# wadx2019/rpo

Measured on AMD Instinct MI355X. Metric: env-steps/sec (whole node), SafeCartpole-v0 (CartSafe-v0) RPODDPG, rollout + one batch-256 constrained policy update per vector step, higher is better.
Workload: dtype f32; 1 GPU; CartSafe-v0 RPODDPG, 4096 vectorised envs per MI355X, scripts/cart_exp.py hyper-parameters, update batch 256 every vector step (reference cadence), replay capacity 20000 per env; envs_per_gpu=4096, global_envs=4096, update_batch=256, hip_graph=True, training_batch_projection=row-wise, rccl_ranks=0, collectives_in_graph=False, graphs_replayed_on_all_ranks=True, graph_capture_fell_back_to_eager=False

## Files before the change

### include/rpo_hip.h

```cpp
#ifndef RPO_HIP_H
#define RPO_HIP_H

#ifdef __cplusplus
extern "C" {
#endif

#define RPO_ABI_VERSION 6

#define RPO_ERR_ARG (-1)
#define RPO_ERR_NULL (-2)

#define RPO_CART_STATE_DIM 6
#define RPO_CART_ACTION_DIM 2
#define RPO_CART_INEQ 6
#define RPO_CART_ROW 24
#define RPO_CART_RING 32
#define RPO_CART_CONSTS_LEN 35

#define RPO_PEND_INTERNAL_DIM 4
#define RPO_PEND_OBS_DIM 5
#define RPO_PEND_ACTION_DIM 2
#define RPO_PEND_ROW 16
#define RPO_PEND_RING 16

// ... 64 lines not shown
#define RPO_EVAL_LEN_SHIFT 2
#define RPO_EVAL_LANE_STEPS 4194304
#define RPO_EVOPF_EVAL_LANE_STEPS 12288

#define RPO_TRACE_ALIGN 4
#define RPO_TRACE_TAIL 4
#define RPO_TRACE_REWARD 0
#define RPO_TRACE_DONE 1
#define RPO_TRACE_INEQ 2
#define RPO_TRACE_EQ 3
#define RPO_TRACE_MAX_BYTES 1073741824

#define RPO_CON_ALIGN 4

#define RPO_CURVE_LEN 16
#define RPO_CURVE_STEP 0
#define RPO_CURVE_EPISODES 1
#define RPO_CURVE_STATS 2
#define RPO_CURVE_LENGTH 12
#define RPO_CURVE_VIOL_STEPS 13
#define RPO_CURVE_NONFINITE 14
#define RPO_CURVE_WS 4096
#define RPO_CURVE_MAX_EPISODES 1048576

#define RPO_NOISE_NONE 0
#define RPO_NOISE_EXPLICIT 1
#define RPO_NOISE_PHILOX 2
#define RPO_NOISE_UNIFORM 3
#define RPO_NOISE_CLIP_ONLY 4

#define RPO_STREAM_RESET 1
#define RPO_STREAM_ACT 2
#define RPO_STREAM_SAMPLE 3
#define RPO_STREAM_POLICY 4
#define RPO_STREAM_EVOPF_DEMAND 5
#define RPO_STREAM_EVOPF_PRICE 6
#define RPO_STREAM_EVAL_OBS 7
#define RPO_STREAM_EVOPF_DAY 8

int rpo_abi_version(void);

#define RPO_TUNE_FWD_STREAM 0
#define RPO_TUNE_FWD_STREAM_WAVES 1
#define RPO_TUNE_BWD_ONEPASS 2
#define RPO_TUNE_GEMM_KSPLIT 3
#define RPO_TUNE_MLP_GEMM 4
#define RPO_TUNE_ROLLOUT_WIDE 5
#define RPO_ROLLOUT_STREAM_FROM 65536
#define RPO_TUNE_BWD_STREAM 6
#define RPO_TUNE_L1_MFMA 7
#define RPO_TUNE_EVOPF_PLACE 8
#define RPO_TUNE_FWD_BF16X3 9
#define RPO_TUNE_COUNT 10
int rpo_tuning(int key, int value);

int rpo_philox_fill(int n, unsigned* out, unsigned long long seed, unsigned id_base, unsigned index,
                    unsigned stream_tag, void* stream);

int rpo_philox_normal(int n, float* out, unsigned long long seed, unsigned id_base, unsigned salt,
                      unsigned stream_tag, const long long* ctrl, void* stream);


int rpo_cartsafe_reset(int n_envs, float* state, int* ep_len, float* ep_ret, const unsigned* ep_count,
                       unsigned long long seed, unsigned env_id_base, void* stream);

int rpo_cartsafe_step(int n_envs, float* state, const float* action, int* ep_len, float* ep_ret, unsigned* ep_count,
                      float* rows, long long cap_steps, float* stats, int stats_cap, long long* ctrl,
                      const float* consts_host, int partial, int max_episode_steps, int auto_reset,
                      float viol_thresh, unsigned long long seed, unsigned env_id_base, void* stream);

int rpo_cartsafe_act_project(int n, const float* ap_raw, const float* noise, float* action, int* iters,
                             int noise_mode, float eps_start, float eps_end, float eps_decay, float box_lo,
                             float box_hi, int max_steps, float corr_lr, float corr_eps, float corr_momentum,
                             const float* consts_host, int partial, unsigned long long seed, unsigned env_id_base,
                             const long long* ctrl, float* stats, int stats_cap, void* stream);

int rpo_cartsafe_complete_bwd(int n, const float* grad_action, float* grad_ap, const float* consts_host,
                              int partial, void* stream);

int rpo_cartsafe_resid(int n, const float* action, float* eq_resid, float* ineq_resid, const float* consts_host,
                       int partial, void* stream);

int rpo_cartsafe_ineq_partial_grad(int n, const float* action, float* step, const float* consts_host, int partial,
                                   void* stream);

int rpo_cartsafe_lagrangian(int n, const float* action, const float* nu, float scale, float* loss_out,
                            float* grad_action, float* grad_nu, const float* consts_host, int partial, void* stream);

int rpo_pendulum_reset(int n_envs, float* internal, float* obs, int* ep_len, float* ep_ret, const unsigned* ep_count,
                       unsigned long long seed, unsigned env_id_base, void* stream);

int rpo_pendulum_step(int n_envs, float* internal, float* obs, const float* action, int* ep_len, float* ep_ret,
                      unsigned* ep_count, float* rows, long long cap_steps, float* stats, int stats_cap,
                      long long* ctrl, int max_episode_steps, int auto_reset, float viol_thresh,
                      unsigned long long seed, unsigned env_id_base, void* stream);

int rpo_pendulum_act_project(int n, const float* obs, int obs_stride, const float* ap_raw, const float* noise,
                             float* action, int* iters, int noise_mode, float eps_start, float eps_end,
                             float eps_decay, float box_lo, float box_hi, int max_steps, float corr_lr,
                             float corr_eps, float corr_momentum, unsigned long long seed, unsigned env_id_base,
                             const long long* ctrl, float* stats, int stats_cap, void* stream);

#define RPO_PROJ_WS_WORDS 5408
#define RPO_PROJ_WS_GAVE_UP 529
int rpo_pendulum_project_batchref(int n, const float* obs, int obs_stride, const float* ap, float* action,
                                  int* iters_out, int max_steps, float corr_lr, float corr_eps, float corr_momentum,
// ... 524 lines not shown
```

### rpo_amd/csrc/common.h

```cpp
#pragma once
#include <hip/hip_runtime.h>
#include <stdint.h>

#include "../../include/rpo_hip.h"

#define RPO_BLOCK 256
#define RPO_WAVE 64
#define RPO_MAX_GRID 2048

#define RPO_LAUNCH_CHECK()                        \
    do {                                          \
        hipError_t e__ = hipGetLastError();       \
        if (e__ != hipSuccess) return (int)e__;   \
    } while (0)

extern int g_rpo_tune[RPO_TUNE_COUNT];
static inline int rpo_tune(int key) { return g_rpo_tune[key]; }

__device__ __forceinline__ float rpo_relu_bits(float x) {
    const int b = __float_as_int(x);
    return __int_as_float(b > 0 ? b : 0);
}

__device__ __forceinline__ float rpo_relu(float x) { return __builtin_elementwise_maximum(x, 0.0f); }

static inline int rpo_cu_count() {
    static int cached[64] = {0};
    int dev = 0;
    if (hipGetDevice(&dev) != hipSuccess || dev < 0 || dev >= 64) return 256;
    if (cached[dev] == 0) {
        int v = 0;
        cached[dev] = (hipDeviceGetAttribute(&v, hipDeviceAttributeMultiprocessorCount, dev) == hipSuccess && v > 0) ? v : 256;
    }
    return cached[dev];
}

static inline int rpo_grid_for(long long n, int per_block = RPO_BLOCK) {
    long long g = (n + per_block - 1) / per_block;
    if (g < 1) g = 1;
    if (g > RPO_MAX_GRID) g = RPO_MAX_GRID;
    return (int)g;
}

struct rpo_u4 {
    uint32_t x, y, z, w;
};

__host__ __device__ __forceinline__ rpo_u4 rpo_philox(uint64_t seed, uint32_t id, uint32_t index, uint32_t stream,
                                                       uint32_t sub = 0u) {
    uint32_t c0 = id, c1 = index, c2 = stream, c3 = sub;
    uint32_t k0 = (uint32_t)seed, k1 = (uint32_t)(seed >> 32);
#pragma unroll
    for (int r = 0; r < 10; ++r) {
        const uint64_t p0 = (uint64_t)0xD2511F53u * c0;
        const uint64_t p1 = (uint64_t)0xCD9E8D57u * c2;
        const uint32_t n0 = (uint32_t)(p1 >> 32) ^ c1 ^ k0;
        const uint32_t n1 = (uint32_t)p1;
        const uint32_t n2 = (uint32_t)(p0 >> 32) ^ c3 ^ k1;
        const uint32_t n3 = (uint32_t)p0;
        c0 = n0; c1 = n1; c2 = n2; c3 = n3;
        k0 += 0x9E3779B9u;
        k1 += 0xBB67AE85u;
    }
    return rpo_u4{c0, c1, c2, c3};
}

__host__ __device__ __forceinline__ float rpo_u01(uint32_t x) { return (float)(x >> 8) * 5.9604644775390625e-08f; }

__device__ __forceinline__ float rpo_normal(uint32_t a, uint32_t b) {
// ... 196 lines not shown
```

### rpo_amd/csrc/nsplit.hip

```cpp
#include <stdlib.h>

#include "cartsafe_dev.h"
#include "heads_dev.h"
#include "host_glue.h"
#include "mlp_bwd.h"
#include "nsplit_dev.h"
#include "pendulum_dev.h"
#include "rollout_args.h"
#include "rollout_env.h"

namespace {

using namespace rpo_mlp_dev;
using namespace rpo_host;

bool split_ok(const Mlp& m) {
    return m.E == 128 && m.H == 256 && !m.cat && m.hd <= 1 && m.S <= 6 && m.A <= 4 && m.n_out >= 1 && m.n_out <= 2 && m.Ws && m.W0 &&
           m.W1 && (m.A == 0 || m.Wa) && (m.n_out == 1 || m.W1b);
}

struct NsBlock { int tile, g; };
__device__ __forceinline__ NsBlock ns_block() {
    const int lin = (int)blockIdx.x + (int)gridDim.x * (int)blockIdx.y, T = (int)gridDim.y;
    return NsBlock{lin % T, lin / T};
// ... 669 lines not shown
        for (int c0 = b_lo; !two && c0 < b_hi; c0 += 64) {
            float hv[64], d0[64];
#pragma unroll
            for (int u = 0; u < 64; ++u) {
                const int bb = c0 + u < b_hi ? c0 + u : b_hi - 1;
                hv[u] = h1[(size_t)bb * H + j];
                d0[u] = dglob[(size_t)bb * dstride];
            }
#pragma unroll
            for (int u = 0; u < 64; ++u) {
                const bool ok = c0 + u < b_hi;
                const float h = ok ? hv[u] : 0.0f, a0 = ok ? d0[u] : 0.0f;
                gb0 += ns_dh(h, a0, 0.0f, w1a, w1b);
                const float hr = fmaxf(h, 0.0f);
                gw1a = fmaf(a0, hr, gw1a);
                gw1b = fmaf(0.0f, hr, gw1b);
            }
        }
        for (int c0 = b_lo; two && c0 < b_hi; c0 += 32) {
            float hv[32], d0[32], d1[32];
#pragma unroll
            for (int u = 0; u < 32; ++u) {
                const int bb = c0 + u < b_hi ? c0 + u : b_hi - 1;
                hv[u] = h1[(size_t)bb * H + j];
                d0[u] = dglob[(size_t)bb * dstride];
                d1[u] = two ? dglob[(size_t)bb * dstride + 1] : 0.0f;
            }
#pragma unroll
            for (int u = 0; u < 32; ++u) {
                const bool ok = c0 + u < b_hi;
                const float h = ok ? hv[u] : 0.0f, a0 = ok ? d0[u] : 0.0f, a1 = ok ? d1[u] : 0.0f;
                gb0 += ns_dh(h, a0, a1, w1a, w1b);
                const float hr = fmaxf(h, 0.0f);
                gw1a = fmaf(a0, hr, gw1a);
                gw1b = fmaf(a1, hr, gw1b);
            }
        }
        partial[part][0][o] = gb0; partial[part][1][o] = gw1a; partial[part][2][o] = gw1b;
    }
    __syncthreads();
    if (tid < 16) {
        const int o = tid, j = rb * 16 + o;
        const float nb0 = cur_b0 + (((partial[0][0][o] + partial[1][0][o]) + partial[2][0][o]) + partial[3][0][o]);
        const float nw1 = cur_w1 + (((partial[0][1][o] + partial[1][1][o]) + partial[2][1][o]) + partial[3][1][o]);
        gr.b0[j] = nb0;
        gr.W1[j] = nw1;
        gmax = fmaxf(fabsf(nb0), fabsf(nw1));
        if (two) {
            const float nw1b = cur_w1b + (((partial[0][2][o] + partial[1][2][o]) + partial[2][2][o]) + partial[3][2][o]);
            gr.W1b[j] = nw1b;
            gmax = fmaxf(gmax, fabsf(nw1b));
        }
    }
    if (rb == 0) {
        __syncthreads();
        float s0 = 0.0f, s1 = 0.0f;
        for (int b2 = tid; b2 < B; b2 += kThreads) {
            s0 += dglob[(size_t)b2 * dstride];
            if (two) s1 += dglob[(size_t)b2 * dstride + 1];
        }
        { float ss[2] = {s0, s1}; rpo_wave_reduce_many(ss, 0u); s0 = ss[0]; s1 = ss[1]; }
        float* red = smem + 256;
        if ((tid & 63) == 0) { red[(tid >> 6) * 2] = s0; red[(tid >> 6) * 2 + 1] = s1; }
        __syncthreads();
        if (tid == 0) {
            const float nb1 = cur_b1 + (((red[0] + red[2]) + red[4]) + red[6]);
            gr.b1[0] = nb1;
            gmax = fmaxf(gmax, fabsf(nb1));
            if (two) {
                const float nb1b = cur_b1b + (((red[1] + red[3]) + red[5]) + red[7]);
                gr.b1b[0] = nb1b;
                gmax = fmaxf(gmax, fabsf(nb1b));
            }
        }
    }
    return gmax;
}

__device__ __forceinline__ float ns_weight_role(const Mlp& net, const MlpGrad& gr, const float* h1, const float* x0,
                                                const float* dglob, int dstride, bool two, int B, int w, float* smem) {
    if (w < kW0Tiles) return ns_dw0_tile(net, gr.W0, h1, x0, dglob, dstride, two, B, w, smem);
    return ns_hv_block(net, gr, h1, dglob, dstride, two, B, w - kW0Tiles, smem);
}

constexpr int kBwdASmem = kRows * (256 + 4) + 16 + 4 * 16 * 16;

template <class L>
__device__ __forceinline__ void bwd_a_role(const SplitArgs& p, float* smem, int b, unsigned fused_consumers = 0u,
                                           unsigned fused_need = 0u, unsigned fused_need_critics = 0u) {
    constexpr int EIN = 128, H = 256, LDH = H + 4;
    const int T = (p.B + kRows - 1) / kRows, B = p.B;
    const int tid = threadIdx.x, lane = tid & 63, wave = tid >> 6, li = lane & 15, lg = lane >> 4;
    {
        const int k = b / (T * kNsGroups), rem = b - k * T * kNsGroups, g = rem / T, tile = rem - g * T;
        const int row0 = tile * kRows;
        const Mlp& net = p.critic[k];
        float* dh_s = smem;
        float* dq_s = smem + kRows * LDH;
        float* wpart = dq_s + 16;
        const int jw = wave * (H / 4), e = g * 16 + li;
        float wv[H / 16], hv[kRows];
#pragma unroll
        for (int ks = 0; ks < H / 16; ++ks) wv[ks] = net.W0[(size_t)(jw + ks * 4 + lg) * EIN + e];
        const float w1a = net.W1[tid];
        if (fused_consumers && fused_need_critics)
            ns_tile_wait(p.tile_sync + (T + tile) * kNsSyncStride, fused_need_critics, p.tile_sync + 3 * T * kNsSyncStride, 16);
#pragma unroll
        for (int r = 0; r < kRows; ++r) hv[r] = row0 + r < B ? p.h1[k][(size_t)(row0 + r) * H + tid] : 0.0f;
        const size_t xo = (size_t)(row0 + (tid >> 4)) * EIN + g * 16 + (tid & 15);
        const float x0v = row0 + (tid >> 4) < B ? p.x0[k][xo] : 0.0f;
        if (fused_consumers) {
            ns_tile_wait(p.tile_sync + (T + tile) * kNsSyncStride, fused_need, p.tile_sync + 3 * T * kNsSyncStride);
            ns_tile_passed(p.tile_sync, T, tile, fused_consumers);
        }
        if (tid < 64) {
            float dq = 0.0f, hub = 0.0f;
            if (tid < kRows && row0 + tid < B) {
                dq = ns_td_row<L>(p, k, row0 + tid, &hub);
                if (g == 0) p.dq[k][row0 + tid] = dq;
            }
            if (tid < kRows) dq_s[tid] = dq;
            const float sum = rpo_row16_sum_desc_lane0(hub);
            if (tid == 0 && g == 0) p.loss_partial[k * T + tile] = sum;
        }
        __syncthreads();
#pragma unroll
        for (int r = 0; r < kRows; ++r) dh_s[r * LDH + tid] = (hv[r] > 0.0f) ? dq_s[r] * w1a : 0.0f;
        __syncthreads();
        f32x4 acc = f32x4{0.0f, 0.0f, 0.0f, 0.0f};
#pragma unroll
        for (int ks = 0; ks < H / 16; ++ks) acc = mfma4(dh_s[li * LDH + jw + ks * 4 + lg], wv[ks], acc);
#pragma unroll
        for (int i = 0; i < 4; ++i) wpart[(wave * 16 + lg * 4 + i) * 16 + li] = acc[i];
        __syncthreads();
        {
            const int r = tid >> 4, ee = tid & 15;
            float v = wpart[(0 * 16 + r) * 16 + ee];
            v = wpart[(1 * 16 + r) * 16 + ee] + v;
            v = wpart[(2 * 16 + r) * 16 + ee] + v;
            v = wpart[(3 * 16 + r) * 16 + ee] + v;
            if (row0 + r < B) p.dx0[k][xo] = x0v > 0.0f ? v : 0.0f;
        }
    }
}

template <class L>
__global__ __launch_bounds__(kThreads) void split_critic_bwd_a_kernel(SplitArgs p) {
    __shared__ __attribute__((aligned(16))) float smem[kBwdASmem];
    bwd_a_role<L>(p, smem, blockIdx.x);
}

__device__ __forceinline__ void adam_prepare(int* step_dev, float beta1, float beta2) {
    const int s = step_dev[0] + 1;
    double* cache = reinterpret_cast<double*>(step_dev + 4);
    cache[0] = 1.0 - pow((double)beta1, (double)s);
    cache[1] = sqrt(1.0 - pow((double)beta2, (double)s));
    step_dev[1] = s;
    step_dev[0] = s;
}

__device__ __forceinline__ void bwd_b_bookkeeping(const SplitArgs& p) {
    if (threadIdx.x != 0) return;
    if (p.prep_step) adam_prepare(p.prep_step, p.prep_beta1, p.prep_beta2);
    if (p.clock_out) p.clock_out[0] += 1;
    if (p.updates_out) p.updates_out[RPO_CTRL_UPDATES] += 1;
}

template <class L>
__device__ __forceinline__ void bwd_b_role(const SplitArgs& p, float* smem, int bx, int k, int own_blocks) {
    if ((p.prep_step || p.clock_out || p.updates_out) && bx == own_blocks - 1) {
        if (k == 0) bwd_b_bookkeeping(p);
        return;
    }
    if (bx < kWeightBlocks) {
        gradmax_flush(p.gradmax, ns_weight_role(p.critic[k], p.critic_grad[k], p.h1[k], p.x0[k], p.dq[k], 1, false, p.B, bx, smem));
        return;
    }
    BwdArgs a{};
    a.net = p.critic[k];
    a.g = p.critic_grad[k];
    a.n = p.B;
    a.s = p.batch_out; a.s_stride = L::ROW;
    a.a = p.batch_out + L::A_OFF; a.a_stride = L::ROW;
    a.dx0 = p.dx0[k];
    a.param_grads = 1;
    a.first_layer_state_only = 0;
    gradmax_flush(p.gradmax, mlp_bwd_first_layer<128>(a, bx - kWeightBlocks));
}

template <class L>
__global__ __launch_bounds__(kThreads) void split_critic_bwd_b_kernel(SplitArgs p) {
    __shared__ __attribute__((aligned(16))) float smem[4 * 16 * 16];
    bwd_b_role<L>(p, smem, blockIdx.x, blockIdx.y, gridDim.x);
}

template <class L>
__global__ __launch_bounds__(kThreads) void split_critic_bwd_b_ride_kernel(SplitArgs p, CartConsts c, RideArgs<typename L::Env> r,
                                                                           int own_blocks) {
    __shared__ __attribute__((aligned(16))) float smem[4 * 16 * 16];
    if ((int)blockIdx.x < own_blocks) bwd_b_role<L>(p, smem, blockIdx.x, blockIdx.y, own_blocks);
    else if (blockIdx.y == 0) ride_tail<typename L::Env>(r, c, smem, blockIdx.x - own_blocks, gridDim.x - own_blocks);
}

}

extern "C" {

int rpo_mlp_split_supported(const rpo_mlp* net) { return net && split_ok(to_dev(net)) ? 1 : 0; }

int rpo_mlp_forward_split(int k, const rpo_mlp* const* nets, int n, const float* const* s, const int* s_stride,
                          const float* const* a, const int* a_stride, float* const* part, float* const* x0_save,
                          float* const* h1_save, void* stream) {
    if (k < 1 || k > 4 || n <= 0 || !nets || !s || !part) return RPO_ERR_ARG;
    SplitFwdArgs4 all{};
    for (int i = 0; i < k; ++i) {
        if (!nets[i] || !s[i] || !part[i]) return RPO_ERR_NULL;
        const Mlp m = to_dev(nets[i]);
        if (!split_ok(m) || (m.A > 0 && (!a || !a[i]))) return RPO_ERR_ARG;
        all.net[i] = SplitFwdArgs{m, n, s[i], s_stride[i], m.A > 0 ? a[i] : nullptr, m.A > 0 ? a_stride[i] : 0, part[i],
                                  x0_save ? x0_save[i] : nullptr, h1_save ? h1_save[i] : nullptr};
    }
    hipLaunchKernelGGL(mlp_forward_split_kernel, dim3(kNsGroups, (n + kRows - 1) / kRows, k), dim3(kNsThreads), 0,
                       (hipStream_t)stream, all);
    RPO_LAUNCH_CHECK();
    return 0;
}

int rpo_mlp_split_head(const rpo_mlp* net, int n, const float* part, float* out, int out_mode, float scale, float base,
                       void* stream) {
    if (!net || !part || !out || n <= 0) return RPO_ERR_NULL;
    const Mlp m = to_dev(net);
    if (!split_ok(m)) return RPO_ERR_ARG;
    hipLaunchKernelGGL(mlp_split_head_kernel, dim3((n * m.n_out + RPO_BLOCK - 1) / RPO_BLOCK), dim3(RPO_BLOCK), 0,
                       (hipStream_t)stream, m, n, part, out, out_mode, scale, base);
    RPO_LAUNCH_CHECK();
    return 0;
}

}

namespace {

struct CartPol {
    typedef CartRow L;
    static constexpr int NI = 6;
    __device__ static __forceinline__ float2 complete(const CartConsts& c, const float* obs, int i, float ap, long long t) {
        rpo_cart_dev::ActArgs a{};
        a.noise_mode = RPO_NOISE_NONE; a.max_steps = 0;
        int k;
        return rpo_cart_dev::cart_explore_project(a, c, i, ap, 0.0f, t, k);
    }
    __device__ static __forceinline__ float lagr(const CartConsts& c, float a0, float a1, const float* nu_p, float scale,
                                                 float (&dist)[6], float2& g) {
// ... 575 lines not shown
            v = wpart[(3 * 16 + r) * 16 + ee] + v;
            if (xlive) {
                v = x0v > 0.0f ? v : 0.0f;
                if (p.shared_embedding) v += cdx;
                p.dx0_a[xo] = v;
            }
        }
    }
}

constexpr int kPolDSmem = kRows * (256 + 4) + 32 + 4 * 16 * 16;

template <class ENV>
__global__ __launch_bounds__(kThreads) void split_policy_d_kernel(SplitArgs p, CartConsts c) {
    __shared__ __attribute__((aligned(16))) float smem[kPolDSmem];
    pol_d_role<ENV>(p, c, smem, blockIdx.x);
}

constexpr int kPolFrontSmem = kPolDSmem > kFrontSmem ? kPolDSmem : kFrontSmem;

template <class ENV>
__global__ __launch_bounds__(kThreads) void split_policy_front_kernel(SplitArgs p, CartConsts c, int with_a) {
    typedef typename ENV::L L;
    __shared__ __attribute__((aligned(16))) float smem[kPolFrontSmem];
    const int K = p.twin ? 2 : 1, T = (int)gridDim.y, z = (int)blockIdx.z;
    const int lin = (int)blockIdx.x + (int)gridDim.x * (int)blockIdx.y;
    const unsigned consumers = (unsigned)(kNsGroups * (K * (1 + with_a) + 1));
    if (z == with_a + 2 * K) {
        pol_d_role<ENV>(p, c, smem, lin, consumers, with_a ? (unsigned)kNsGroups : 0u, (unsigned)(kNsGroups * K));
        return;
    }
    if (z >= with_a + K) {
        pol_c_role(p, smem, (z - with_a - K) * T * kNsGroups + lin, consumers, (unsigned)(kNsGroups * K));
        ns_tile_arrive(p.tile_sync + (lin % T) * kNsSyncStride, 1u << 16);
        return;
    }
    if (threadIdx.x >= kNsThreads) return;
    NsLds<128>& lds = *reinterpret_cast<NsLds<128>*>(smem);
    float4* tile = reinterpret_cast<float4*>(reinterpret_cast<char*>(smem) + sizeof(NsLds<128>));
    const NsBlock nb = ns_block();
    unsigned* sync = p.tile_sync;
    if (z < with_a) {
        pol_a_role<L>(p, lds, tile, nb.tile * kRows, nb.g);
        ns_tile_arrive(sync + nb.tile * kNsSyncStride);
    } else {
        pol_b_role<ENV>(p, c, lds, tile, nb.tile, nb.g, z - with_a, with_a ? sync + nb.tile * kNsSyncStride : nullptr,
                        (unsigned)kNsGroups);
        ns_tile_arrive(sync + (T + nb.tile) * kNsSyncStride);
        if (with_a) ns_tile_passed(sync, T, nb.tile, consumers);
    }
}

template <class ENV>
__global__ __launch_bounds__(kThreads) void split_policy_e_kernel(SplitArgs p, int fl_blocks) {
    typedef typename ENV::L L;
    __shared__ __attribute__((aligned(16))) float smem[4 * 16 * 16];
    if (blockIdx.x < kWeightBlocks) {
        gradmax_flush(p.gradmax, ns_weight_role(p.actor, p.actor_grad, p.h1_a, p.x0_a, p.dout, 2, p.actor.n_out > 1, p.B,
                                                blockIdx.x, smem));
        return;
    }
    const int fb = blockIdx.x - kWeightBlocks;
    if (fb == fl_blocks) {
        const int tid = threadIdx.x, T = (p.B + kRows - 1) / kRows;
        if (tid < 8) {
            float sacc = 0.0f;
            for (int g = 0; g < T; ++g) sacc += p.lag_partial[g * 8 + tid];
            const float inv_b = 1.0f / (float)p.B;
            if (tid == 0) p.lag_out[0] = inv_b * sacc;
            else if (tid == 7) { if (!p.twin) p.lag_out[1] = inv_b * sacc; }
            else if (tid - 1 < ENV::NI) p.nu_grad[tid - 1] += inv_b * sacc;
        }
        if (tid >= 64 && tid < 67 && p.prep2_step[tid - 64]) adam_prepare(p.prep2_step[tid - 64], p.prep2_beta1[tid - 64], p.prep2_beta2[tid - 64]);
        if (tid == 128 && p.clock_out) p.clock_out[0] += 1;
        if (tid == 192 && p.updates_out) p.updates_out[RPO_CTRL_UPDATES] += 1;
        return;
    }
    BwdArgs a{};
    a.net = p.actor;
    a.g = p.actor_grad;
    a.n = p.B;
    a.s = p.batch_out; a.s_stride = L::ROW;
    a.dx0 = p.dx0_a;
    a.param_grads = 1;
    gradmax_flush(p.gradmax, mlp_bwd_first_layer<128>(a, fb));
}

}

namespace {

enum : unsigned {
    kNeedPolicy = 1u,
    kNeedCritics = 2u, kNeedTargets = 4u, kNeedCriticGrads = 8u, kNeedActorGrad = 16u,
    kNeedActor = 32u,
};

int to_args(const rpo_split_update* u, unsigned need, SplitArgs& a, CartConsts& c) {
    if (!u) return RPO_ERR_NULL;
    if (u->batch <= 0 || u->batch > kBwdMaxB || (u->env != 0 && u->env != 1)) return RPO_ERR_ARG;
    const int S = u->env == 0 ? 6 : 5, K = u->twin ? 2 : 1;
    a = SplitArgs{};
    a.twin = u->twin ? 1 : 0; a.B = u->batch;
    auto ok_actor = [&](const rpo_mlp* h, Mlp& m) {
        if (!h) return (int)RPO_ERR_NULL;
        m = to_dev(h);
        return (split_ok(m) && m.S == S && m.A == 0 && m.n_out == (u->twin ? 2 : 1)) ? 0 : (int)RPO_ERR_ARG;
    };
    auto ok_critic = [&](const rpo_mlp* h, Mlp& m) {
        if (!h) return (int)RPO_ERR_NULL;
        m = to_dev(h);
        return (split_ok(m) && m.S == S && m.A == 2 && m.n_out == 1) ? 0 : (int)RPO_ERR_ARG;
    };
    if (need & kNeedPolicy) {
        if (int e = u->twin ? ok_actor(u->actor, a.actor) : ok_actor(u->actor_target, a.actor_target)) return e;
    }
    if (need & kNeedActor) {
        if (int e = ok_actor(u->actor, a.actor)) return e;
    }
    if (need & kNeedCritics) {
        if (int e = ok_critic(u->critic1, a.critic[0])) return e;
        if (K == 2) if (int e = ok_critic(u->critic2, a.critic[1])) return e;
    }
    if (need & kNeedTargets) {
        if (int e = ok_critic(u->critic_target1, a.critic_target[0])) return e;
        if (K == 2) if (int e = ok_critic(u->critic_target2, a.critic_target[1])) return e;
    }
    if (need & kNeedCriticGrads) {
        if (!u->critic1_grad || (K == 2 && !u->critic2_grad)) return RPO_ERR_NULL;
        a.critic_grad[0] = grad_dev(u->critic1_grad);
// ... 174 lines not shown
int fused_args(const rpo_split_update* u, const rpo_rollout_rider* r, Variant v, int env, unsigned need, SplitArgs& a, CartConsts& c) {
    if (int e = ride_checks(u, r, v, true)) return e;
    if (!u) return RPO_ERR_NULL;
    if (u->env != env) return RPO_ERR_ARG;
    return to_args(u, need | actor_need(v), a, c);
}

dim3 fused_grid(const SplitArgs& a, const rpo_rollout_rider* r, Variant v, int planes) {
    return slab_grid(a, planes + (v == kRide ? ride_planes(r, tiles(a.B), 2) : (int)(v == kPol)));
}

int front(const rpo_split_update* u, const rpo_rollout_rider* r, Variant v, void* stream) {
    SplitArgs a; CartConsts c;
    if (int e = fused_args(u, r, v, 0, kNeedPolicy | kNeedCritics | kNeedTargets, a, c)) return e;
    if (!a.batch_out || !a.ctrl || !a.part_pi || !a.tile_sync) return RPO_ERR_NULL;
    if (int e = sample_check(a, RPO_ERR_NULL)) return e;
    if ((a.twin && !a.logp) || a.max_steps < 0 || !a.loss_partial || !critic_bufs(a, kBufAll)) return RPO_ERR_NULL;
    if (int e = pol_check(u, a, v)) return e;
    const dim3 grid = fused_grid(a, r, v, 1 + 3 * critics(a));
    if (v == kRide) return launch(kFrontRide, grid, kThreads, 0, stream, a, c, Ride{a, r});
    return launch(kFront, grid, kThreads, 0, stream, a, c, (int)(v == kPol));
}

int mid(const rpo_split_update* u, const rpo_rollout_rider* r, Variant v, void* stream) {
    SplitArgs a; CartConsts c;
    if (int e = fused_args(u, r, v, 1, kNeedCritics | kNeedTargets, a, c)) return e;
    if (!a.batch_out || !a.ctrl || !a.next_actions || !a.tile_sync || !a.loss_partial || (a.twin && !a.logp) || !critic_bufs(a, kBufAll))
        return RPO_ERR_NULL;
    if (int e = pol_check(u, a, v)) return e;
    const dim3 grid = fused_grid(a, r, v, 2 * critics(a));
    if (v == kRide) return launch(kMidRide, grid, kThreads, 0, stream, a, c, Ride{a, r});
    return launch(kMid, grid, kThreads, 0, stream, a, c, (int)(v == kPol));
}

int pfront(const rpo_split_update* u, const rpo_rollout_rider* r, Variant v, void* stream) {
    SplitArgs a; CartConsts c;
    if (int e = fused_args(u, r, v, 1, kNeedPolicy | kNeedCritics | kNeedTargets, a, c)) return e;
    if (!a.batch_out || !a.ctrl || !a.part_pi || !a.next_actions || !a.tile_sync || !a.loss_partial || !u->proj_ws || (a.twin && !a.logp))
        return RPO_ERR_NULL;
    if (int e = sample_check(a, RPO_ERR_ARG)) return e;
    if (a.max_steps < 0 || !proj_multi_fits(a.B, a.max_steps) || !proj_ws_ok(u->proj_ws, u->proj_store_mode)) return RPO_ERR_ARG;
    if (!critic_bufs(a, kBufAll)) return RPO_ERR_NULL;
    if (int e = pol_check(u, a, v)) return e;
    const dim3 grid = fused_grid(a, r, v, 2 + 3 * critics(a));
    if (v == kRide) return launch(kPfrontRide, grid, kThreads, 0, stream, a, c, Ride{a, r}, u->proj_ws, u->proj_store_mode);
    return launch(kPfront, grid, kThreads, 0, stream, a, c, (int)(v == kPol), u->proj_ws, u->proj_store_mode);
}

int bwd_b(const rpo_split_update* u, const rpo_rollout_rider* r, Variant v, void* stream) {
    SplitArgs a; CartConsts c;
    if (int e = ride_checks(u, r, v, false)) return e;
    if (int e = to_args(u, kNeedCritics | kNeedCriticGrads | actor_need(v), a, c)) return e;
    if (!a.batch_out || !critic_bufs(a, kBufBwd)) return RPO_ERR_NULL;
    const int own = bwd_b_blocks(a);
    if (v == kRide)
        return launch_env(kBwdBRide, u->env, dim3(own + (r->n_envs + kThreads - 1) / kThreads, critics(a)), kThreads, stream, a, c,
                          Ride{a, r}, own);
    return launch_env(kBwdB, u->env, dim3(own, critics(a)), kThreads, stream, a);
}

int policy_b(const rpo_split_update* u, int fused, int with_a, void* stream) {
    SplitArgs a; CartConsts c;
    if (int e = to_args(u, kNeedActor | kNeedCritics, a, c)) return e;
    if (!a.batch_out || !a.ctrl || (!a.part_pi && !a.part_pol) || !a.nu || !a.noise_out || !a.actions || !a.g_act || !a.lag_partial ||
        (a.twin ? (!a.raw || !a.logp) : !a.ap_det) || !critic_bufs(a, kBufFwd))
        return RPO_ERR_NULL;
    if (!fused) return launch_env(kPolicyB, u->env, slab_grid(a, critics(a)), kNsThreads, stream, a, c);
    if (!a.tile_sync || !a.da_part || !critic_bufs(a, kBufDx0) || !a.dx0_a || !a.dout || !a.x0_a || !a.h1_a) return RPO_ERR_NULL;
    return launch_env(kPolicyFront, u->env, slab_grid(a, with_a + 2 * critics(a) + 1), kThreads, stream, a, c, with_a);
}

}

extern "C" {

int rpo_split_critic_fwd_a(const rpo_split_update* u, void* stream) { return fwd_a(u, nullptr, kPlain, stream); }
int rpo_split_critic_fwd_a_ride(const rpo_split_update* u, const rpo_rollout_rider* r, void* stream) { return fwd_a(u, r, kRide, stream); }

int rpo_split_critic_fwd_b(const rpo_split_update* u, void* stream) { return fwd_b(u, nullptr, kPlain, stream); }
int rpo_split_critic_fwd_b_pol(const rpo_split_update* u, void* stream) { return fwd_b(u, nullptr, kPol, stream); }
int rpo_split_critic_fwd_b_ride(const rpo_split_update* u, const rpo_rollout_rider* r, void* stream) { return fwd_b(u, r, kRide, stream); }

int rpo_split_critic_front(const rpo_split_update* u, void* stream) { return front(u, nullptr, kPlain, stream); }
int rpo_split_critic_front_pol(const rpo_split_update* u, void* stream) { return front(u, nullptr, kPol, stream); }
int rpo_split_critic_front_ride(const rpo_split_update* u, const rpo_rollout_rider* r, void* stream) { return front(u, r, kRide, stream); }

int rpo_split_critic_mid(const rpo_split_update* u, void* stream) { return mid(u, nullptr, kPlain, stream); }
int rpo_split_critic_mid_pol(const rpo_split_update* u, void* stream) { return mid(u, nullptr, kPol, stream); }
int rpo_split_critic_mid_ride(const rpo_split_update* u, const rpo_rollout_rider* r, void* stream) { return mid(u, r, kRide, stream); }

int rpo_split_critic_pfront(const rpo_split_update* u, void* stream) { return pfront(u, nullptr, kPlain, stream); }
int rpo_split_critic_pfront_pol(const rpo_split_update* u, void* stream) { return pfront(u, nullptr, kPol, stream); }
int rpo_split_critic_pfront_ride(const rpo_split_update* u, const rpo_rollout_rider* r, void* stream) { return pfront(u, r, kRide, stream); }

int rpo_split_critic_bwd_b(const rpo_split_update* u, void* stream) { return bwd_b(u, nullptr, kPlain, stream); }
int rpo_split_critic_bwd_b_ride(const rpo_split_update* u, const rpo_rollout_rider* r, void* stream) { return bwd_b(u, r, kRide, stream); }

int rpo_split_policy_b(const rpo_split_update* u, void* stream) { return policy_b(u, 0, 0, stream); }
int rpo_split_policy_front(const rpo_split_update* u, void* stream) { return policy_b(u, 1, 1, stream); }
int rpo_split_policy_front_bc(const rpo_split_update* u, void* stream) { return policy_b(u, 1, 0, stream); }

int rpo_split_critic_bwd_a(const rpo_split_update* u, void* stream) {
    SplitArgs a; CartConsts c;
    if (int e = to_args(u, kNeedCritics | kNeedTargets, a, c)) return e;
    if (!a.batch_out || !a.loss_partial || (a.twin && !a.logp) || !critic_bufs(a, kBufAll)) return RPO_ERR_NULL;
    return launch_env(kBwdA, u->env, dim3(critics(a) * tiles(a.B) * kNsGroups), kThreads, stream, a);
}

int rpo_split_pend_head_project(const rpo_split_update* u, void* stream) {
    SplitArgs a; CartConsts c;
    if (int e = to_args(u, kNeedPolicy, a, c)) return e;
    if (u->env != 1 || a.max_steps < 0) return RPO_ERR_ARG;
    if (!a.batch_out || !a.ctrl || !a.part_pi || !a.next_actions || (a.twin && !a.logp)) return RPO_ERR_NULL;
    static_assert(kPmWords == RPO_PROJ_WS_WORDS && kPmGaveUp == RPO_PROJ_WS_GAVE_UP, "workspace layout");
    if (u->proj_ws && proj_multi_fits(a.B, a.max_steps))
        return project_multi(a, u->proj_ws, u->proj_store_mode, nullptr, nullptr, 0, stream);
    if (a.B <= 256) return launch(split_pend_head_project_wide_kernel, dim3(1), 1024, 0, stream, a);
    return launch(kProjectTall, dim3(1), (a.B + RPO_WAVE - 1) / RPO_WAVE * RPO_WAVE, ((size_t)a.B + 4) * sizeof(float), stream, a);
}

int rpo_pendulum_project_batchref_ws(int n, const float* obs, int obs_stride, const float* ap, float* action, int* iters_out,
                                     int max_steps, float corr_lr, float corr_eps, float corr_momentum,
                                     unsigned long long* ws, int store_mode, void* stream) {
    if (n <= 0 || max_steps < 0 || !proj_multi_fits(n, max_steps) || obs_stride < RPO_PEND_OBS_DIM) return RPO_ERR_ARG;
    if (!obs || !ap || !action || !ws) return RPO_ERR_NULL;
    SplitArgs a{};
    a.B = n; a.next_actions = action; a.proj_iters = iters_out; a.max_steps = max_steps; a.corr_lr = corr_lr;
    a.corr_eps = corr_eps; a.corr_momentum = corr_momentum;
    return project_multi(a, ws, store_mode, ap, obs, obs_stride, stream);
}

int rpo_split_policy_a(const rpo_split_update* u, void* stream) {
    SplitArgs a; CartConsts c;
    if (int e = to_args(u, kNeedActor, a, c)) return e;
    if (!a.batch_out || (!a.part_pi && !a.part_pol) || !a.x0_a || !a.h1_a) return RPO_ERR_NULL;
    return launch_env(kPolicyA, u->env, dim3(kNsGroups, tiles(a.B)), kNsThreads, stream, a);
}

int rpo_split_policy_c(const rpo_split_update* u, void* stream) {
    SplitArgs a; CartConsts c;
    if (int e = to_args(u, kNeedCritics, a, c)) return e;
    if (!a.da_part || !a.lag_partial || (a.twin && !a.logp) || !critic_bufs(a, kBufFwd | kBufDx0)) return RPO_ERR_NULL;
    return launch(split_policy_c_kernel, dim3(critics(a) * tiles(a.B) * kNsGroups), kThreads, 0, stream, a);
}

int rpo_split_policy_d(const rpo_split_update* u, void* stream) {
    SplitArgs a; CartConsts c;
    if (int e = to_args(u, kNeedActor | kNeedActorGrad, a, c)) return e;
    if (!a.batch_out || !a.ctrl || !a.da_part || !a.g_act || !a.noise_out || !a.x0_a || !a.h1_a || !a.dx0_a || !a.dout ||
        (a.twin ? !a.raw : !a.ap_det) || (a.shared_embedding && !critic_bufs(a, kBufDx0)))
        return RPO_ERR_NULL;
    return launch_env(kPolicyD, u->env, dim3(tiles(a.B) * kNsGroups), kThreads, stream, a, c);
}

int rpo_split_policy_e(const rpo_split_update* u, void* stream) {
    SplitArgs a; CartConsts c;
    if (int e = to_args(u, kNeedActor | kNeedActorGrad, a, c)) return e;
    if (!a.batch_out || !a.dx0_a || !a.lag_partial || !a.lag_out || !a.nu_grad || !a.dout || !a.x0_a || !a.h1_a) return RPO_ERR_NULL;
    const int fl_blocks = mlp_fl_blocks(a.actor.E * (a.actor.S + 1));
    return launch_env(kPolicyE, u->env, dim3(kWeightBlocks + fl_blocks + 1), kThreads, stream, a, fl_blocks);
}

int rpo_xcc_probe(int gx, int gy, int gz, int threads, int* out, void* stream) {
    if (gx <= 0 || gy <= 0 || gz <= 0 || threads <= 0 || threads > 1024) return RPO_ERR_ARG;
    if (!out) return RPO_ERR_NULL;
    return launch(xcc_probe_kernel, dim3(gx, gy, gz), threads, 0, stream, out);
}

int rpo_hw_probe(int gx, int gy, int gz, int threads, int lds_bytes, int spin, int* out, void* stream) {
    if (gx <= 0 || gy <= 0 || gz <= 0 || threads <= 0 || threads > 1024 || lds_bytes < 4 || lds_bytes > 65536 || spin < 0) return RPO_ERR_ARG;
    if (!out) return RPO_ERR_NULL;
    return launch(hw_probe_kernel, dim3(gx, gy, gz), threads, lds_bytes, stream, out, spin);
}

}
```

### rpo_amd/csrc/train_ops.hip

```cpp
#include <stdlib.h>
#include "common.h"
#include "heads_dev.h"

namespace {

__global__ __launch_bounds__(RPO_BLOCK) void td_huber_kernel(
    int n, const float* __restrict__ q1, const float* __restrict__ q2, const float* __restrict__ qn1,
    const float* __restrict__ qn2, const float* __restrict__ logp, float alpha, const float* __restrict__ reward,
    int reward_stride, const float* __restrict__ done, int done_stride, float gamma, float* __restrict__ loss_out,
    float* __restrict__ grad_q1, float* __restrict__ grad_q2, float* __restrict__ target_out) {
    __shared__ float red[RPO_BLOCK / RPO_WAVE];
    const float inv_n = 1.0f / (float)n;
    float acc = 0.0f;
    for (int i = blockIdx.x * RPO_BLOCK + threadIdx.x; i < n; i += gridDim.x * RPO_BLOCK) {
        const float qn = rpo_head_dev::td_next_value(qn1[i], qn2 ? qn2[i] : 0.0f, qn2 != nullptr,
                                                     logp ? logp[i] : 0.0f, logp != nullptr, alpha);
        const float y = rpo_head_dev::td_target(reward[(size_t)i * reward_stride], done[(size_t)i * done_stride], gamma,
                                                qn);
        if (target_out) target_out[i] = y;
        float h1 = 0.0f, h2 = 0.0f;
        const float g1 = rpo_head_dev::td_huber_row(q1[i], y, inv_n, &h1);
        if (grad_q1) grad_q1[i] = g1;
        if (q2) {
            const float g2 = rpo_head_dev::td_huber_row(q2[i], y, inv_n, &h2);
// ... 134 lines not shown
            cache[1] = sqrt(1.0 - pow((double)p.beta2, (double)(step + 1)));
            p.step_dev[1] = step + 1;
            if (p.reset_gradmax && p.gradmax)
                for (int j = 0; j < RPO_GRADMAX_SLOTS; ++j) p.gradmax[j * (RPO_GRADMAX_LEN / RPO_GRADMAX_SLOTS)] = 0.0f;
            if (p.clock) p.clock[0] += 1;
        }
    }
}

__global__ __launch_bounds__(RPO_BLOCK) void adam_kernel(AdamArgs p) { adam_body(p); }

struct AdamArgs4 {
    AdamArgs seg[4];
};
__global__ __launch_bounds__(RPO_BLOCK) void adam_multi_kernel(AdamArgs4 p) { adam_body(p.seg[blockIdx.y]); }

__global__ __launch_bounds__(RPO_BLOCK) void min_q_bwd_kernel(int n, const float* __restrict__ q1, const float* __restrict__ q2,
                                                              float scale, float* __restrict__ dq1, float* __restrict__ dq2) {
    for (int i = blockIdx.x * RPO_BLOCK + threadIdx.x; i < n; i += gridDim.x * RPO_BLOCK) {
        const float a = q1[i], b = q2[i];
        const float w = (a < b ? 1.0f : 0.0f) + 0.5f * (a == b ? 1.0f : 0.0f);
        dq1[i] = w * scale;
        dq2[i] = (1.0f - w) * scale;
    }
}

__global__ __launch_bounds__(RPO_BLOCK) void polyak_kernel(long long n, const float* __restrict__ param,
                                                           float* __restrict__ target, float tau) {
    for (long long i = (long long)blockIdx.x * RPO_BLOCK + threadIdx.x; i < n; i += (long long)gridDim.x * RPO_BLOCK)
        target[i] = target[i] * (1.0f - tau) + param[i] * tau;
}

__global__ __launch_bounds__(RPO_BLOCK) void philox_fill_kernel(int n, uint32_t* __restrict__ out, uint64_t seed,
                                                                uint32_t id_base, uint32_t index, uint32_t tag) {
    for (int i = blockIdx.x * RPO_BLOCK + threadIdx.x; i < n; i += gridDim.x * RPO_BLOCK) {
        const rpo_u4 r = rpo_philox(seed, id_base + (uint32_t)i, index, tag);
        reinterpret_cast<uint4*>(out)[i] = make_uint4(r.x, r.y, r.z, r.w);
    }
}

__global__ __launch_bounds__(RPO_BLOCK) void philox_normal_kernel(int n, float* __restrict__ out, uint64_t seed,
                                                                  uint32_t id_base, uint32_t salt, uint32_t tag,
                                                                  const long long* __restrict__ ctrl) {
    const uint32_t t = ctrl ? (uint32_t)ctrl[RPO_CTRL_T] : 0u;
    const uint32_t sub = ctrl ? (uint32_t)ctrl[RPO_CTRL_UPDATES] : 0u;
    for (int i = blockIdx.x * RPO_BLOCK + threadIdx.x; i < n; i += gridDim.x * RPO_BLOCK) {
        const rpo_u4 r = rpo_philox(seed, id_base + (uint32_t)i, t + salt, tag, sub);
        out[i] = rpo_normal(r.x, r.y);
    }
}

}

int g_rpo_tune[RPO_TUNE_COUNT] = { 1,  16,  1,  1,
                                   1,  2,  1,
                                   1,  0,  0};

extern "C" {

int rpo_philox_normal(int n, float* out, unsigned long long seed, unsigned id_base, unsigned salt,
                      unsigned stream_tag, const long long* ctrl, void* stream) {
    if (n <= 0) return RPO_ERR_ARG;
    if (!out) return RPO_ERR_NULL;
    hipLaunchKernelGGL(philox_normal_kernel, dim3(rpo_grid_for(n)), dim3(RPO_BLOCK), 0, (hipStream_t)stream, n, out,
                       (uint64_t)seed, (uint32_t)id_base, (uint32_t)salt, (uint32_t)stream_tag, ctrl);
    RPO_LAUNCH_CHECK();
    return 0;
}

int rpo_abi_version(void) { return RPO_ABI_VERSION; }

int rpo_tuning(int key, int value) {
    if (key < 0 || key >= RPO_TUNE_COUNT) return RPO_ERR_ARG;
    const int old = g_rpo_tune[key];
    if (value >= 0) g_rpo_tune[key] = value;
    return old;
}

int rpo_philox_fill(int n, unsigned* out, unsigned long long seed, unsigned id_base, unsigned index,
                    unsigned stream_tag, void* stream) {
    if (n <= 0) return RPO_ERR_ARG;
    if (!out) return RPO_ERR_NULL;
    hipLaunchKernelGGL(philox_fill_kernel, dim3(rpo_grid_for(n)), dim3(RPO_BLOCK), 0, (hipStream_t)stream, n, out,
                       (uint64_t)seed, (uint32_t)id_base, (uint32_t)index, (uint32_t)stream_tag);
    RPO_LAUNCH_CHECK();
    return 0;
}

int rpo_td_huber(int n, const float* q1, const float* q2, const float* qn1, const float* qn2, const float* logp,
                 float alpha, const float* reward, int reward_stride, const float* done, int done_stride, float gamma,
                 float* loss_out, float* grad_q1, float* grad_q2, float* target_out, void* stream) {
    if (n <= 0 || reward_stride <= 0 || done_stride <= 0) return RPO_ERR_ARG;
    if (!q1 || !qn1 || !reward || !done) return RPO_ERR_NULL;
    hipLaunchKernelGGL(td_huber_kernel, dim3(rpo_grid_for(n)), dim3(RPO_BLOCK), 0, (hipStream_t)stream, n, q1, q2, qn1,
                       qn2, logp, alpha, reward, reward_stride, done, done_stride, gamma, loss_out, grad_q1, grad_q2,
                       target_out);
    RPO_LAUNCH_CHECK();
    return 0;
}

int rpo_absmax(long long n, const float* x, float* max_out, void* stream) {
    if (n <= 0) return RPO_ERR_ARG;
    if (!x || !max_out) return RPO_ERR_NULL;
    if ((reinterpret_cast<uintptr_t>(x) & 15u) != 0) return RPO_ERR_ARG;
    hipLaunchKernelGGL(absmax_kernel, dim3(rpo_grid_for(n / 4 + 1)), dim3(RPO_BLOCK), 0, (hipStream_t)stream, n, x,
                       max_out, 0);
    RPO_LAUNCH_CHECK();
    return 0;
}

int rpo_absmax_slots(long long n, const float* x, float* gradmax, void* stream) {
    if (n <= 0) return RPO_ERR_ARG;
    if (!x || !gradmax) return RPO_ERR_NULL;
    if ((reinterpret_cast<uintptr_t>(x) & 15u) != 0) return RPO_ERR_ARG;
    hipLaunchKernelGGL(absmax_kernel, dim3(rpo_grid_for(n / 4 + 1)), dim3(RPO_BLOCK), 0, (hipStream_t)stream, n, x,
                       gradmax, 1);
    RPO_LAUNCH_CHECK();
    return 0;
}

int rpo_adam_step(long long n, float* param, float* grad, float* exp_avg, float* exp_avg_sq, int* step_dev,
                  float lr, float beta1, float beta2, float eps, float weight_decay, int maximize, float clip_thres,
                  float* gradmax, int reset_gradmax, int zero_grad, int clamp_min0, float* target, float tau,
                  long long* clock, int prepared, void* stream) {
    if (n <= 0) return RPO_ERR_ARG;
    if (!param || !grad || !exp_avg || !exp_avg_sq || !step_dev) return RPO_ERR_NULL;
// ... 54 lines not shown
```

Baseline: 101.5 million env-steps/s.

## Stage hidden-vector weight-gradient reduction through shared memory with prefetched tiles

```diff
diff --git a/include/rpo_hip.h b/include/rpo_hip.h
--- a/include/rpo_hip.h
+++ b/include/rpo_hip.h
@@ -140,6 +140,7 @@
 #define RPO_TUNE_EVOPF_PLACE 8
 #define RPO_TUNE_FWD_BF16X3 9
 #define RPO_TUNE_COUNT 10
+#define RPO_TUNE_WGRAD_STAGED 11
 int rpo_tuning(int key, int value);
 
 int rpo_philox_fill(int n, unsigned* out, unsigned long long seed, unsigned id_base, unsigned index,
diff --git a/rpo_amd/csrc/common.h b/rpo_amd/csrc/common.h
--- a/rpo_amd/csrc/common.h
+++ b/rpo_amd/csrc/common.h
@@ -14,7 +14,8 @@
         if (e__ != hipSuccess) return (int)e__;   \
     } while (0)
 
-extern int g_rpo_tune[RPO_TUNE_COUNT];
+constexpr int kRpoTuneSlots = RPO_TUNE_WGRAD_STAGED + 1;
+extern int g_rpo_tune[kRpoTuneSlots];
 static inline int rpo_tune(int key) { return g_rpo_tune[key]; }
 
 __device__ __forceinline__ float rpo_relu_bits(float x) {
diff --git a/rpo_amd/csrc/nsplit.hip b/rpo_amd/csrc/nsplit.hip
--- a/rpo_amd/csrc/nsplit.hip
+++ b/rpo_amd/csrc/nsplit.hip
@@ -745,7 +745,7 @@
             gmax = fmaxf(gmax, fabsf(nw1b));
         }
     }
-    if (rb == 0) {
+    if (rb == 0 && !(RPO_NS_SKIP & 4)) {
         __syncthreads();
         float s0 = 0.0f, s1 = 0.0f;
         for (int b2 = tid; b2 < B; b2 += kThreads) {
@@ -770,10 +770,169 @@
     return gmax;
 }
 
+constexpr int kHvRows = 64;
+constexpr int kHvLdPart = kHvRows * 16 + 16;
+constexpr int kHvLdD = kHvRows + 4;
+constexpr int kHvSmem = 4 * kHvLdPart + 2 * 4 * kHvLdD + 4 * 3 * 16 + 8;
+constexpr int kWeightSmem = kHvSmem > 4 * 16 * 16 ? kHvSmem : 4 * 16 * 16;
+
+struct HvStage { f32x4 h[4]; float d0, d1; };
+
+__device__ __forceinline__ void ns_hv_stage_load(HvStage& s, const float* __restrict__ h1, const float* dglob, int dstride, bool two,
+                                                 int B, int rb, int c0) {
+    constexpr int H = 256;
+    const int tid = threadIdx.x, r = tid >> 2, q = tid & 3, last = B - 1;
+#pragma unroll
+    for (int part = 0; part < 4; ++part) {
+        const int bb = (int)(((long long)B * part) / 4) + c0 + r, bc = bb < last ? bb : last;
+        s.h[part] = *reinterpret_cast<const f32x4*>(&h1[(size_t)bc * H + rb * 16 + q * 4]);
+    }
+    const int bb = (int)(((long long)B * (tid >> 6)) / 4) + c0 + (tid & 63), bc = bb < last ? bb : last;
+    s.d0 = dglob[(size_t)bc * dstride];
+    s.d1 = two ? dglob[(size_t)bc * dstride + 1] : 0.0f;
+}
+
+template <bool TWO, int N>
+__device__ __forceinline__ void ns_hv_chain(const float* hcol, const float* dr0, const float* dr1, int len, float w1a, float w1b,
+                                            float& gb0, float& gw1a, float& gw1b) {
+    static_assert(N % 4 == 0, "16-byte reads of the d values");
+    float hl[N], a0l[N], a1l[N];
+#pragma unroll
+    for (int u = 0; u < N; ++u) hl[u] = hcol[u * 16];
+#pragma unroll
+    for (int u = 0; u < N; u += 4) {
+        const f32x4 v0 = *reinterpret_cast<const f32x4*>(&dr0[u]);
+        f32x4 v1 = f32x4{0.0f, 0.0f, 0.0f, 0.0f};
+        if (TWO) v1 = *reinterpret_cast<const f32x4*>(&dr1[u]);
+#pragma unroll
+        for (int i = 0; i < 4; ++i) { a0l[u + i] = v0[i]; a1l[u + i] = v1[i]; }
+    }
+#pragma unroll
+    for (int u = 0; u < N; ++u) {
+        const bool ok = u < len;
+        const float h = ok ? hl[u] : 0.0f, a0 = ok ? a0l[u] : 0.0f, a1 = (TWO && ok) ? a1l[u] : 0.0f;
+        gb0 += ns_dh(h, a0, a1, w1a, w1b);
+        const float hr = fmaxf(h, 0.0f);
+        gw1a = fmaf(a0, hr, gw1a);
+        gw1b = fmaf(a1, hr, gw1b);
+    }
+}
+
+__device__ __forceinline__ float ns_hv_block_staged(const Mlp& net, const MlpGrad& gr, const float* __restrict__ h1,
+                                                    const float* dglob, int dstride, bool two, int B, int rb, float* smem) {
+    static_assert(kBwdMaxB <= 4 * kThreads, "db1: at most four rows per thread");
+    const int tid = threadIdx.x;
+    float* hs = smem;
+    float* d0s = smem + 4 * kHvLdPart;
+    float* d1s = d0s + 4 * kHvLdD;
+    float (*partial)[3][16] = reinterpret_cast<float (*)[3][16]>(d1s + 4 * kHvLdD);
+    float* red = d1s + 4 * kHvLdD + 4 * 3 * 16;
+    float gmax = 0.0f;
+    float cur_b0 = 0.0f, cur_w1 = 0.0f, cur_w1b = 0.0f, cur_b1 = 0.0f, cur_b1b = 0.0f;
+    if (tid < 16) {
+        cur_b0 = gr.b0[rb * 16 + tid];
+        cur_w1 = gr.W1[rb * 16 + tid];
+        if (two) cur_w1b = gr.W1b[rb * 16 + tid];
+    }
+    if (rb == 0 && tid == 0) {
+        cur_b1 = gr.b1[0];
+        if (two) cur_b1b = gr.b1b[0];
+    }
+    const int o = tid & 15, part = (tid >> 4) & 3;
+    const int b_lo = (int)(((long long)B * part) / 4), b_hi = (int)(((long long)B * (part + 1)) / 4);
+    float w1a = 0.0f, w1b = 0.0f;
+    if (tid < 64) {
+        w1a = net.W1[rb * 16 + o];
+        if (two) w1b = net.W1b[rb * 16 + o];
+    }
+    float dv0[4] = {0.0f, 0.0f, 0.0f, 0.0f}, dv1[4] = {0.0f, 0.0f, 0.0f, 0.0f};
+    const bool db1 = rb == 0 && !(RPO_NS_SKIP & 4);
+    if (db1) {
+#pragma unroll
+        for (int i = 0; i < 4; ++i) {
+            const int b2 = tid + i * kThreads, bc = b2 < B ? b2 : B - 1;
+            dv0[i] = dglob[(size_t)bc * dstride];
+            if (two) dv1[i] = dglob[(size_t)bc * dstride + 1];
+        }
+    }
+    HvStage st;
+    ns_hv_stage_load(st, h1, dglob, dstride, two, B, rb, 0);
+    if (db1) {
+        float s0 = 0.0f, s1 = 0.0f;
+#pragma unroll
+        for (int i = 0; i < 4; ++i) {
+            if (tid + i * kThreads < B) {
+                s0 += dv0[i];
+                if (two) s1 += dv1[i];
+            }
+        }
+        { float ss[2] = {s0, s1}; rpo_wave_reduce_many(ss, 0u); s0 = ss[0]; s1 = ss[1]; }
+        if ((tid & 63) == 0) { red[(tid >> 6) * 2] = s0; red[(tid >> 6) * 2 + 1] = s1; }
+    }
+    float gb0 = 0.0f, gw1a = 0.0f, gw1b = 0.0f;
+    const int nmax = (B + 3) / 4;
+    for (int c0 = 0;;) {
+#pragma unroll
+        for (int pp = 0; pp < 4; ++pp) *reinterpret_cast<f32x4*>(&hs[pp * kHvLdPart + tid * 4]) = st.h[pp];
+        d0s[(tid >> 6) * kHvLdD + (tid & 63)] = st.d0;
+        if (two) d1s[(tid >> 6) * kHvLdD + (tid & 63)] = st.d1;
+        __syncthreads();
+        if (tid < 64) {
+            const int len = b_hi - b_lo - c0;
+            const float* hcol = hs + part * kHvLdPart + o;
+            const float* dr0 = d0s + part * kHvLdD;
+            const float* dr1 = d1s + part * kHvLdD;
+            if (two) {
+                ns_hv_chain<true, kHvRows / 2>(hcol, dr0, dr1, len, w1a, w1b, gb0, gw1a, gw1b);
+                ns_hv_chain<true, kHvRows / 2>(hcol + kHvRows / 2 * 16, dr0 + kHvRows / 2, dr1 + kHvRows / 2, len - kHvRows / 2, w1a,
+                                               w1b, gb0, gw1a, gw1b);
+            } else {
+                ns_hv_chain<false, kHvRows>(hcol, dr0, dr1, len, w1a, w1b, gb0, gw1a, gw1b);
+            }
+        }
+        c0 += kHvRows;
+        if (c0 >= nmax) break;
+        __syncthreads();
+        ns_hv_stage_load(st, h1, dglob, dstride, two, B, rb, c0);
+    }
+    if (tid < 64) { partial[part][0][o] = gb0; partial[part][1][o] = gw1a; partial[part][2][o] = gw1b; }
+    __syncthreads();
+    if (tid < 16) {
+        const int j = rb * 16 + o;
+        const float nb0 = cur_b0 + (((partial[0][0][o] + partial[1][0][o]) + partial[2][0][o]) + partial[3][0][o]);
+        const float nw1 = cur_w1 + (((partial[0][1][o] + partial[1][1][o]) + partial[2][1][o]) + partial[3][1][o]);
+        gr.b0[j] = nb0;
+        gr.W1[j] = nw1;
+        gmax = fmaxf(fabsf(nb0), fabsf(nw1));
+        if (two) {
+            const float nw1b = cur_w1b + (((partial[0][2][o] + partial[1][2][o]) + partial[2][2][o]) + partial[3][2][o]);
+            gr.W1b[j] = nw1b;
+            gmax = fmaxf(gmax, fabsf(nw1b));
+        }
+    }
+    if (db1 && tid == 0) {
+        const float nb1 = cur_b1 + (((red[0] + red[2]) + red[4]) + red[6]);
+        gr.b1[0] = nb1;
+        gmax = fmaxf(gmax, fabsf(nb1));
+        if (two) {
+            const float nb1b = cur_b1b + (((red[1] + red[3]) + red[5]) + red[7]);
+            gr.b1b[0] = nb1b;
+            gmax = fmaxf(gmax, fabsf(nb1b));
+        }
+    }
+    return gmax;
+}
+
 __device__ __forceinline__ float ns_weight_role(const Mlp& net, const MlpGrad& gr, const float* h1, const float* x0,
-                                                const float* dglob, int dstride, bool two, int B, int w, float* smem) {
-    if (w < kW0Tiles) return ns_dw0_tile(net, gr.W0, h1, x0, dglob, dstride, two, B, w, smem);
+                                                const float* dglob, int dstride, bool two, int B, int w, float* smem, bool staged) {
+    if (w < kW0Tiles) return (RPO_NS_SKIP & 32) ? 0.0f : ns_dw0_tile(net, gr.W0, h1, x0, dglob, dstride, two, B, w, smem);
+    if (RPO_NS_SKIP & 2) return 0.0f;
+    if (staged) return ns_hv_block_staged(net, gr, h1, dglob, dstride, two, B, w - kW0Tiles, smem);
     return ns_hv_block(net, gr, h1, dglob, dstride, two, B, w - kW0Tiles, smem);
+}
+
+bool wgrad_staged(const float* h1_0, const float* h1_1) {
+    return rpo_tune(RPO_TUNE_WGRAD_STAGED) != 0 && !(((uintptr_t)h1_0 | (uintptr_t)h1_1) & 15u);
 }
 
 constexpr int kBwdASmem = kRows * (256 + 4) + 16 + 4 * 16 * 16;
@@ -860,15 +1019,17 @@
 }
 
 template <class L>
-__device__ __forceinline__ void bwd_b_role(const SplitArgs& p, float* smem, int bx, int k, int own_blocks) {
+__device__ __forceinline__ void bwd_b_role(const SplitArgs& p, float* smem, int bx, int k, int own_blocks, bool staged) {
     if ((p.prep_step || p.clock_out || p.updates_out) && bx == own_blocks - 1) {
-        if (k == 0) bwd_b_bookkeeping(p);
+        if (k == 0 && !(RPO_NS_SKIP & 8)) bwd_b_bookkeeping(p);
         return;
     }
     if (bx < kWeightBlocks) {
-        gradmax_flush(p.gradmax, ns_weight_role(p.critic[k], p.critic_grad[k], p.h1[k], p.x0[k], p.dq[k], 1, false, p.B, bx, smem));
+        gradmax_flush(p.gradmax, ns_weight_role(p.critic[k], p.critic_grad[k], p.h1[k], p.x0[k], p.dq[k], 1, false, p.B, bx, smem,
+                                                staged));
         return;
     }
+    if (RPO_NS_SKIP & 64) return;
     BwdArgs a{};
     a.net = p.critic[k];
     a.g = p.critic_grad[k];
@@ -882,16 +1043,16 @@
 }
 
 template <class L>
-__global__ __launch_bounds__(kThreads) void split_critic_bwd_b_kernel(SplitArgs p) {
-    __shared__ __attribute__((aligned(16))) float smem[4 * 16 * 16];
-    bwd_b_role<L>(p, smem, blockIdx.x, blockIdx.y, gridDim.x);
+__global__ __launch_bounds__(kThreads) void split_critic_bwd_b_kernel(SplitArgs p, int staged) {
+    __shared__ __attribute__((aligned(16))) float smem[kWeightSmem];
+    bwd_b_role<L>(p, smem, blockIdx.x, blockIdx.y, gridDim.x, staged != 0);
 }
 
 template <class L>
 __global__ __launch_bounds__(kThreads) void split_critic_bwd_b_ride_kernel(SplitArgs p, CartConsts c, RideArgs<typename L::Env> r,
                                                                            int own_blocks) {
     __shared__ __attribute__((aligned(16))) float smem[4 * 16 * 16];
-    if ((int)blockIdx.x < own_blocks) bwd_b_role<L>(p, smem, blockIdx.x, blockIdx.y, own_blocks);
+    if ((int)blockIdx.x < own_blocks) bwd_b_role<L>(p, smem, blockIdx.x, blockIdx.y, own_blocks, false);
     else if (blockIdx.y == 0) ride_tail<typename L::Env>(r, c, smem, blockIdx.x - own_blocks, gridDim.x - own_blocks);
 }
 
@@ -1573,30 +1734,42 @@
 }
 
 template <class ENV>
-__global__ __launch_bounds__(kThreads) void split_policy_e_kernel(SplitArgs p, int fl_blocks) {
+__global__ __launch_bounds__(kThreads) void split_policy_e_kernel(SplitArgs p, int fl_blocks, int staged) {
     typedef typename ENV::L L;
-    __shared__ __attribute__((aligned(16))) float smem[4 * 16 * 16];
+    __shared__ __attribute__((aligned(16))) float smem[kWeightSmem];
     if (blockIdx.x < kWeightBlocks) {
         gradmax_flush(p.gradmax, ns_weight_role(p.actor, p.actor_grad, p.h1_a, p.x0_a, p.dout, 2, p.actor.n_out > 1, p.B,
-                                                blockIdx.x, smem));
+                                                blockIdx.x, smem, staged != 0));
         return;
     }
     const int fb = blockIdx.x - kWeightBlocks;
     if (fb == fl_blocks) {
         const int tid = threadIdx.x, T = (p.B + kRows - 1) / kRows;
-        if (tid < 8) {
+        if (tid < 8 && !(RPO_NS_SKIP & 16)) {
             float sacc = 0.0f;
-            for (int g = 0; g < T; ++g) sacc += p.lag_partial[g * 8 + tid];
+            if (staged) {
+                constexpr int kMaxT = kBwdMaxB / kRows;
+                float lv[kMaxT];
+#pragma unroll
+                for (int g = 0; g < kMaxT; ++g) lv[g] = p.lag_partial[(g < T ? g : T - 1) * 8 + tid];
+#pragma unroll
+                for (int g = 0; g < kMaxT; ++g)
+                    if (g < T) sacc += lv[g];
+            } else {
+                for (int g = 0; g < T; ++g) sacc += p.lag_partial[g * 8 + tid];
+            }
             const float inv_b = 1.0f / (float)p.B;
             if (tid == 0) p.lag_out[0] = inv_b * sacc;
             else if (tid == 7) { if (!p.twin) p.lag_out[1] = inv_b * sacc; }
             else if (tid - 1 < ENV::NI) p.nu_grad[tid - 1] += inv_b * sacc;
         }
+        if (RPO_NS_SKIP & 8) return;
         if (tid >= 64 && tid < 67 && p.prep2_step[tid - 64]) adam_prepare(p.prep2_step[tid - 64], p.prep2_beta1[tid - 64], p.prep2_beta2[tid - 64]);
         if (tid == 128 && p.clock_out) p.clock_out[0] += 1;
         if (tid == 192 && p.updates_out) p.updates_out[RPO_CTRL_UPDATES] += 1;
         return;
     }
+    if (RPO_NS_SKIP & 64) return;
     BwdArgs a{};
     a.net = p.actor;
     a.g = p.actor_grad;
@@ -1877,11 +2050,11 @@
     if (int e = ride_checks(u, r, v, false)) return e;
     if (int e = to_args(u, kNeedCritics | kNeedCriticGrads | actor_need(v), a, c)) return e;
     if (!a.batch_out || !critic_bufs(a, kBufBwd)) return RPO_ERR_NULL;
-    const int own = bwd_b_blocks(a);
+    const int own = bwd_b_blocks(a), staged = wgrad_staged(a.h1[0], a.twin ? a.h1[1] : nullptr) ? 1 : 0;
     if (v == kRide)
         return launch_env(kBwdBRide, u->env, dim3(own + (r->n_envs + kThreads - 1) / kThreads, critics(a)), kThreads, stream, a, c,
                           Ride{a, r}, own);
-    return launch_env(kBwdB, u->env, dim3(own, critics(a)), kThreads, stream, a);
+    return launch_env(kBwdB, u->env, dim3(own, critics(a)), kThreads, stream, a, staged);
 }
 
 int policy_b(const rpo_split_update* u, int fused, int with_a, void* stream) {
@@ -1983,7 +2156,8 @@
     if (int e = to_args(u, kNeedActor | kNeedActorGrad, a, c)) return e;
     if (!a.batch_out || !a.dx0_a || !a.lag_partial || !a.lag_out || !a.nu_grad || !a.dout || !a.x0_a || !a.h1_a) return RPO_ERR_NULL;
     const int fl_blocks = mlp_fl_blocks(a.actor.E * (a.actor.S + 1));
-    return launch_env(kPolicyE, u->env, dim3(kWeightBlocks + fl_blocks + 1), kThreads, stream, a, fl_blocks);
+    return launch_env(kPolicyE, u->env, dim3(kWeightBlocks + fl_blocks + 1), kThreads, stream, a, fl_blocks,
+                      wgrad_staged(a.h1_a, nullptr) ? 1 : 0);
 }
 
 int rpo_xcc_probe(int gx, int gy, int gz, int threads, int* out, void* stream) {
diff --git a/rpo_amd/csrc/train_ops.hip b/rpo_amd/csrc/train_ops.hip
--- a/rpo_amd/csrc/train_ops.hip
+++ b/rpo_amd/csrc/train_ops.hip
@@ -210,9 +210,11 @@
 
 }
 
-int g_rpo_tune[RPO_TUNE_COUNT] = { 1,  16,  1,  1,
+int g_rpo_tune[kRpoTuneSlots] = { 1,  16,  1,  1,
                                    1,  2,  1,
-                                   1,  0,  0};
+                                   1,  0,  0,  0,
+                                   1};
+static_assert(RPO_TUNE_COUNT == 10 && RPO_TUNE_WGRAD_STAGED == 11, "the table above follows the keys' indices");
 
 extern "C" {
 
@@ -229,7 +231,7 @@
 int rpo_abi_version(void) { return RPO_ABI_VERSION; }
 
 int rpo_tuning(int key, int value) {
-    if (key < 0 || key >= RPO_TUNE_COUNT) return RPO_ERR_ARG;
+    if (key < 0 || (key >= RPO_TUNE_COUNT && key != RPO_TUNE_WGRAD_STAGED)) return RPO_ERR_ARG;
     const int old = g_rpo_tune[key];
     if (value >= 0) g_rpo_tune[key] = value;
     return old;
```

Result: faster. 104.6 million env-steps/s, median of 6 (+3.0%).
